# IamArmanNikkhah/viewport-entropy-toolkit

Hardware: NVIDIA B200
Metric: user-frame samples/sec (bin+weighted entropy, 200 tiles) (higher is better)
Workload: dtype f64

## Files before the change

viewport_entropy_toolkit_b200/csrc/vet_whist_i8.cuh:

```cuda
#pragma once
#include <cuda.h>

#include "vet_common.cuh"
#include "vet_stream_tma.cuh"

namespace vet {

constexpr int kI8Slices = 5;
constexpr int kI8FracBits = 39;
constexpr int kI8TilesPerBlock = 48;
constexpr int kI8N = kI8Slices * kI8TilesPerBlock;
constexpr int kI8M = 128;
constexpr int kI8BK = 128;
constexpr int kI8Stages = 3;
constexpr int kI8StagesOne = 4;
constexpr int kI8ABytes = kI8M * kI8BK;
constexpr int kI8BBytes = kI8N * kI8BK;
constexpr int kI8StageBytes = 2 * kI8ABytes + kI8BBytes;
constexpr int kI8Threads = 192;
constexpr int kI8MaxSplit = 8;
constexpr int kI8TmemCols = 512;
constexpr int kI8SmemBytes = kI8Stages * kI8StageBytes + 1024;
static_assert(kI8StageBytes % 1024 == 0 && (kI8ABytes + kI8BBytes) % 1024 == 0, "stages must keep the 1024 B swizzle alignment");
static_assert(kI8StagesOne * (kI8ABytes + kI8BBytes) <= kI8Stages * kI8StageBytes, "both layouts share one ring");

__device__ __forceinline__ void tma_load_2d(uint32_t dst, const void* tmap, uint32_t bar, int c0, int c1) {
  asm volatile(
      "cp.async.bulk.tensor.2d.shared::cluster.global.mbarrier::complete_tx::bytes [%0], [%1, {%3, %4}], [%2];" ::"r"(dst),
      "l"(tmap), "r"(bar), "r"(c0), "r"(c1)
      : "memory");
}
__device__ __forceinline__ void tc_fence_before() { asm volatile("tcgen05.fence::before_thread_sync;" ::: "memory"); }
__device__ __forceinline__ void tc_fence_after() { asm volatile("tcgen05.fence::after_thread_sync;" ::: "memory"); }
__device__ __forceinline__ void tc_alloc(uint32_t smem_dst, uint32_t cols) {
  asm volatile("tcgen05.alloc.cta_group::1.sync.aligned.shared::cta.b32 [%0], %1;" ::"r"(smem_dst), "r"(cols) : "memory");
  asm volatile("tcgen05.relinquish_alloc_permit.cta_group::1.sync.aligned;" ::: "memory");
}
__device__ __forceinline__ void tc_dealloc(uint32_t taddr, uint32_t cols) {
  asm volatile("tcgen05.dealloc.cta_group::1.sync.aligned.b32 %0, %1;" ::"r"(taddr), "r"(cols) : "memory");
}
__device__ __forceinline__ void tc_commit(uint32_t bar) {
  asm volatile("tcgen05.commit.cta_group::1.mbarrier::arrive::one.shared::cluster.b64 [%0];" ::"r"(bar) : "memory");
}
__device__ __forceinline__ void tc_mma_i8(uint32_t d, uint64_t adesc, uint64_t bdesc, uint32_t idesc, uint32_t accumulate) {
  asm volatile(
      "{\n"
      ".reg .pred p;\n"
      "setp.ne.b32 p, %4, 0;\n"
      "tcgen05.mma.cta_group::1.kind::i8 [%0], %1, %2, %3, p;\n"
      "}\n" ::"r"(d),
      "l"(adesc), "l"(bdesc), "r"(idesc), "r"(accumulate)
      : "memory");
}
__device__ __forceinline__ void tc_ld16(uint32_t taddr, uint32_t (&r)[16]) {
  asm volatile(
      "tcgen05.ld.sync.aligned.32x32b.x16.b32 {%0, %1, %2, %3, %4, %5, %6, %7, %8, %9, %10, %11, %12, %13, %14, %15}, [%16];"
      : "=r"(r[0]), "=r"(r[1]), "=r"(r[2]), "=r"(r[3]), "=r"(r[4]), "=r"(r[5]), "=r"(r[6]), "=r"(r[7]), "=r"(r[8]), "=r"(r[9]),
        "=r"(r[10]), "=r"(r[11]), "=r"(r[12]), "=r"(r[13]), "=r"(r[14]), "=r"(r[15])
      : "r"(taddr)
      : "memory");
}
__device__ __forceinline__ void tc_wait_ld() { asm volatile("tcgen05.wait::ld.sync.aligned;" ::: "memory"); }

__device__ __forceinline__ uint64_t i8_smem_desc(uint32_t saddr) {
  return (uint64_t)((saddr & 0x3FFFFu) >> 4) | (1ull << 16) | ((uint64_t)(1024 >> 4) << 32) | (1ull << 46) | (2ull << 61);
}
constexpr uint32_t kI8InstrDesc = (2u << 4) | ((uint32_t)(kI8N >> 3) << 17) | ((uint32_t)(kI8M >> 4) << 24);

struct WhistI8Args {
  int64_t F;
  int T;
  int n_blocks;
  int row_a;
  int row_b;
  const uint32_t* flag_b;
  const uint32_t* run_if;
  int shift;
  int accumulate;
  const int2* kb_range;
  double* hist;
  int ksplit;
  int* part;
};

__global__ void __launch_bounds__(kI8Threads, 1)
k_whist_i8(const __grid_constant__ CUtensorMap tm_cnt, const __grid_constant__ CUtensorMap tm_w, WhistI8Args a) {
  const int tile_id = blockIdx.x / a.ksplit;
  const int sp = blockIdx.x % a.ksplit;
  const int nb = tile_id % a.n_blocks;
  const int mb = tile_id / a.n_blocks;
  if (a.run_if && a.run_if[mb] == 0u) return;
  extern __shared__ unsigned char smem_dyn[];
  __shared__ __align__(8) unsigned long long s_full[kI8StagesOne], s_empty[kI8StagesOne], s_accum;
  __shared__ uint32_t s_tmem;
  const int warp = threadIdx.x >> 5, lane = threadIdx.x & 31;
  const uint32_t ring = (smem_u32(smem_dyn) + 1023u) & ~1023u;
  int2 kr = a.kb_range[nb];
  if (a.ksplit > 1) {
    const int per = (kr.y - kr.x + a.ksplit - 1) / a.ksplit;
    kr.x = min(kr.y, kr.x + sp * per);
    kr.y = min(kr.y, kr.x + per);
  }
  const bool two = a.flag_b && a.flag_b[mb] != 0u;

  const uint32_t nstages = two ? kI8Stages : kI8StagesOne;
  const uint32_t stage_bytes = two ? (uint32_t)kI8StageBytes : (uint32_t)(kI8ABytes + kI8BBytes);
  const uint32_t w_off = two ? 2u * kI8ABytes : (uint32_t)kI8ABytes;
  if (threadIdx.x == 0) {
    for (int i = 0; i < kI8StagesOne; ++i) {
      mbar_init(smem_u32(&s_full[i]), 1);
      mbar_init(smem_u32(&s_empty[i]), 1);
    }
    mbar_init(smem_u32(&s_accum), 1);
    asm volatile("fence.mbarrier_init.release.cluster;" ::: "memory");
  }
  if (warp == 1) tc_alloc(smem_u32(&s_tmem), kI8TmemCols);
  tc_fence_before();
  __syncthreads();
  tc_fence_after();
  const uint32_t tmem = s_tmem;

  if (warp == 0) {
    if (lane == 0) {
      uint32_t stage = 0, phase = 0;
      for (int kb = kr.x; kb < kr.y; ++kb) {
        mbar_wait(smem_u32(&s_empty[stage]), phase ^ 1u);
        const uint32_t bar = smem_u32(&s_full[stage]);
        const uint32_t base = ring + stage * stage_bytes;
        mbar_expect_tx(bar, stage_bytes);
        tma_load_2d(base, &tm_cnt, bar, kb * kI8BK, a.row_a + mb * kI8M);
        if (two) tma_load_2d(base + kI8ABytes, &tm_cnt, bar, kb * kI8BK, a.row_b + mb * kI8M);
        tma_load_2d(base + w_off, &tm_w, bar, kb * kI8BK, nb * kI8N);
        if (++stage == nstages) {
          stage = 0;
          phase ^= 1u;
        }
      }
    }
  } else if (warp == 1) {
    if (lane == 0) {
      uint32_t stage = 0, phase = 0;
      for (int kb = kr.x; kb < kr.y; ++kb) {
        mbar_wait(smem_u32(&s_full[stage]), phase);
        tc_fence_after();
        const uint32_t base = ring + stage * stage_bytes;
#pragma unroll
        for (int k = 0; k < kI8BK / 32; ++k) {
          const uint32_t acc = (kb > kr.x || k > 0) ? 1u : 0u;
          const uint64_t bdesc = i8_smem_desc(base + w_off + k * 32);
          tc_mma_i8(tmem, i8_smem_desc(base + k * 32), bdesc, kI8InstrDesc, acc);
          if (two) tc_mma_i8(tmem + 256, i8_smem_desc(base + kI8ABytes + k * 32), bdesc, kI8InstrDesc, acc);
        }
        tc_commit(smem_u32(&s_empty[stage]));
        if (++stage == nstages) {
          stage = 0;
          phase ^= 1u;
        }
      }
      tc_commit(smem_u32(&s_accum));
    }
    __syncwarp();
  } else {
    const int q = warp & 3;
    const int64_t f = (int64_t)mb * kI8M + q * 32 + lane;
    const uint32_t lane_base = tmem + ((uint32_t)(q * 32) << 16);
    if (a.ksplit > 1) {
      int* __restrict__ part = a.part + ((int64_t)tile_id * a.ksplit + sp) * (2 * kI8N * kI8M) + q * 32 + lane;
      const bool have = kr.y > kr.x;
      if (have) {
        mbar_wait(smem_u32(&s_accum), 0u);
        tc_fence_after();
      }
#pragma unroll 1
      for (int c0 = 0; c0 < kI8N; c0 += 16) {
        uint32_t r0[16], r1[16];
#pragma unroll
        for (int j = 0; j < 16; ++j) r0[j] = r1[j] = 0u;
        if (have) {
          tc_ld16(lane_base + c0, r0);
          if (two) tc_ld16(lane_base + 256 + c0, r1);
          tc_wait_ld();
        }
#pragma unroll
        for (int j = 0; j < 16; ++j) {
          __stcg(part + (c0 + j) * kI8M, (int)r0[j]);
          if (two) __stcg(part + (kI8N + c0 + j) * kI8M, (int)r1[j]);
        }
      }
    } else {
      mbar_wait(smem_u32(&s_accum), 0u);
      tc_fence_after();
#pragma unroll 1
      for (int j0 = 0; j0 < kI8TilesPerBlock; j0 += 16) {
        double v[16];
#pragma unroll
        for (int j = 0; j < 16; ++j) v[j] = 0.0;
#pragma unroll
        for (int s = kI8Slices - 1; s >= 0; --s) {
          uint32_t r0[16], r1[16];
          tc_ld16(lane_base + s * kI8TilesPerBlock + j0, r0);
          if (two) tc_ld16(lane_base + 256 + s * kI8TilesPerBlock + j0, r1);
          tc_wait_ld();
          const double scale = __longlong_as_double((long long)(1023 + 8 * s - kI8FracBits + a.shift) << 52);
#pragma unroll
          for (int j = 0; j < 16; ++j) {
            long long x = (long long)(int)r0[j];
            if (two) x += (long long)(int)r1[j] << 8;
            v[j] = fma((double)x, scale, v[j]);
          }
        }
        if (f < a.F) {
          double* __restrict__ row = a.hist + f * (int64_t)a.T;
#pragma unroll
          for (int j = 0; j < 16; ++j) {
            const int tile = nb * kI8TilesPerBlock + j0 + j;
            if (tile < a.T) row[tile] = a.accumulate ? row[tile] + v[j] : v[j];
          }
        }
      }
    }
  }
  tc_fence_before();
  __syncthreads();
  if (warp == 1) tc_dealloc(tmem, kI8TmemCols);
}

__global__ void __launch_bounds__(kI8M) k_whist_i8_finish(WhistI8Args a) {
  const int tile_id = blockIdx.y;
  const int nb = tile_id % a.n_blocks;
  const int mb = tile_id / a.n_blocks;
  if (a.run_if && a.run_if[mb] == 0u) return;
  const int j = blockIdx.x;
  const int tile = nb * kI8TilesPerBlock + j;
  const int64_t f = (int64_t)mb * kI8M + threadIdx.x;
  if (tile >= a.T || f >= a.F) return;
  const bool two = a.flag_b && a.flag_b[mb] != 0u;
  const int* __restrict__ part = a.part + (int64_t)tile_id * a.ksplit * (2 * kI8N * kI8M) + threadIdx.x;
  int x0[kI8Slices], x1[kI8Slices];
#pragma unroll
  for (int s = 0; s < kI8Slices; ++s) x0[s] = x1[s] = 0;
#pragma unroll
  for (int sp = 0; sp < kI8MaxSplit; ++sp) {
    if (sp < a.ksplit) {
#pragma unroll
      for (int s = 0; s < kI8Slices; ++s) {
        const int* p = part + (int64_t)sp * (2 * kI8N * kI8M) + (s * kI8TilesPerBlock + j) * kI8M;
        x0[s] += __ldcg(p);
        if (two) x1[s] += __ldcg(p + kI8N * kI8M);
      }
    }
  }
  double v = 0.0;
#pragma unroll
  for (int s = kI8Slices - 1; s >= 0; --s) {
    long long x = (long long)x0[s];
    if (two) x += (long long)x1[s] << 8;
    const double scale = __longlong_as_double((long long)(1023 + 8 * s - kI8FracBits + a.shift) << 52);
    v = fma((double)x, scale, v);
  }
  double* __restrict__ row = a.hist + f * (int64_t)a.T;
  row[tile] = a.accumulate ? row[tile] + v : v;
}

struct CntPlanesArgs {
  const uint32_t* cnt;
  int64_t F;
  int cpad;
  int kp;
  int64_t plane_stride;
  uint8_t* planes;
  uint8_t* dirty;
  uint32_t* hi1;
  uint32_t* hi2;
};

__global__ void __launch_bounds__(256) k_cnt_planes(CntPlanesArgs a) {
  const int lane = threadIdx.x & 31;
  const int64_t warp = (blockIdx.x * (int64_t)blockDim.x + threadIdx.x) >> 5;
  const int64_t nwarps = ((int64_t)gridDim.x * blockDim.x) >> 5;
  const int upr = a.kp >> 7;
  const int64_t units = a.F * upr;
  uint32_t* __restrict__ p0 = reinterpret_cast<uint32_t*>(a.planes);
  uint32_t* __restrict__ p1 = reinterpret_cast<uint32_t*>(a.planes + a.plane_stride);
  uint32_t* __restrict__ p2 = reinterpret_cast<uint32_t*>(a.planes + 2 * a.plane_stride);
  constexpr int kUnroll = 4;
  for (int64_t u0 = warp * kUnroll; u0 < units; u0 += nwarps * kUnroll) {
    uint4 v[kUnroll];
#pragma unroll
    for (int i = 0; i < kUnroll; ++i) {
      const int64_t u = u0 + i;
      v[i] = make_uint4(0u, 0u, 0u, 0u);
      if (u < units) {
        const int64_t f = u / upr;
        const int c = (int)(u % upr) * 128 + lane * 4;
        if (c < a.cpad) v[i] = __ldg(reinterpret_cast<const uint4*>(a.cnt + f * (int64_t)a.cpad + c));
      }
    }
#pragma unroll
    for (int i = 0; i < kUnroll; ++i) {
      const int64_t u = u0 + i;
      if (u < units) {
        const int64_t f = u / upr;
        const int64_t o = (f * (int64_t)a.kp + (u % upr) * 128) / 4 + lane;
        const uint32_t w1 = pack_bytes(v[i], 8), w2 = pack_bytes(v[i], 16);
        p0[o] = pack_bytes(v[i], 0);
        p1[o] = w1;
        p2[o] = w2;
        if (w1 && *reinterpret_cast<volatile uint32_t*>(&a.hi1[f >> 7]) == 0u) atomicOr(&a.hi1[f >> 7], 1u);
        if (w2 && *reinterpret_cast<volatile uint32_t*>(&a.hi2[f >> 7]) == 0u) atomicOr(&a.hi2[f >> 7], 1u);
        if (u % upr == 0 && lane == 0) a.dirty[f] = 3;
      }
    }
  }
}

}
```

Measured before the change: 418.8 billion.

## Use variable-width tile blocks with sparse k-lists and fused high-plane pass

Replaces fixed 48-tile blocks with per-block descriptors of variable width (up to 51 tiles, N up to 256), choosing a matching weight tensor map per width. K-blocks now come from a sparse kb_list so empty k-chunks are skipped. The high-byte plane is handled as a second pass inside the same kernel, with a TMEM-free barrier, instead of a separate launch with run_if/accumulate. It also adds an optional globaltimer instrumentation path. The cost is per-element tcgen05 loads for unaligned columns and more complex synchronisation.

```diff
diff --git a/viewport_entropy_toolkit_b200/csrc/vet_whist_i8.cuh b/viewport_entropy_toolkit_b200/csrc/vet_whist_i8.cuh
--- a/viewport_entropy_toolkit_b200/csrc/vet_whist_i8.cuh
+++ b/viewport_entropy_toolkit_b200/csrc/vet_whist_i8.cuh
@@ -9,20 +9,33 @@
 constexpr int kI8Slices = 5;
 constexpr int kI8FracBits = 39;
 constexpr int kI8TilesPerBlock = 48;
-constexpr int kI8N = kI8Slices * kI8TilesPerBlock;
+constexpr int kI8MaxTiles = 51;
+constexpr int kI8MaxN = 256;
 constexpr int kI8M = 128;
 constexpr int kI8BK = 128;
 constexpr int kI8Stages = 3;
 constexpr int kI8StagesOne = 4;
 constexpr int kI8ABytes = kI8M * kI8BK;
-constexpr int kI8BBytes = kI8N * kI8BK;
+constexpr int kI8BBytes = kI8MaxN * kI8BK;
 constexpr int kI8StageBytes = 2 * kI8ABytes + kI8BBytes;
 constexpr int kI8Threads = 192;
 constexpr int kI8MaxSplit = 8;
 constexpr int kI8TmemCols = 512;
+constexpr int kI8PartPlane = kI8MaxN * kI8M;
 constexpr int kI8SmemBytes = kI8Stages * kI8StageBytes + 1024;
 static_assert(kI8StageBytes % 1024 == 0 && (kI8ABytes + kI8BBytes) % 1024 == 0, "stages must keep the 1024 B swizzle alignment");
 static_assert(kI8StagesOne * (kI8ABytes + kI8BBytes) <= kI8Stages * kI8StageBytes, "both layouts share one ring");
+static_assert(((kI8Slices * kI8MaxTiles + 15) & ~15) == kI8MaxN, "the widest block fills N = 256");
+
+#ifdef VET_WHIST_I8_CLOCK
+constexpr int kI8ClockSlots = 4096;
+__device__ unsigned long long g_whist_i8_clock[kI8ClockSlots][3];
+__device__ __forceinline__ unsigned long long globaltimer() {
+  unsigned long long t;
+  asm volatile("mov.u64 %0, %globaltimer;" : "=l"(t));
+  return t;
+}
+#endif
 
 __device__ __forceinline__ void tma_load_2d(uint32_t dst, const void* tmap, uint32_t bar, int c0, int c1) {
   asm volatile(
@@ -61,47 +74,73 @@
       : "memory");
 }
 __device__ __forceinline__ void tc_wait_ld() { asm volatile("tcgen05.wait::ld.sync.aligned;" ::: "memory"); }
+__device__ __forceinline__ void tc_ld16_any(uint32_t taddr, uint32_t (&r)[16]) {
+  if ((taddr & 15u) == 0u) {
+    tc_ld16(taddr, r);
+  } else {
+#pragma unroll
+    for (int j = 0; j < 16; ++j)
+      asm volatile("tcgen05.ld.sync.aligned.32x32b.x1.b32 {%0}, [%1];" : "=r"(r[j]) : "r"(taddr + j) : "memory");
+  }
+}
 
 __device__ __forceinline__ uint64_t i8_smem_desc(uint32_t saddr) {
   return (uint64_t)((saddr & 0x3FFFFu) >> 4) | (1ull << 16) | ((uint64_t)(1024 >> 4) << 32) | (1ull << 46) | (2ull << 61);
 }
-constexpr uint32_t kI8InstrDesc = (2u << 4) | ((uint32_t)(kI8N >> 3) << 17) | ((uint32_t)(kI8M >> 4) << 24);
+__device__ __forceinline__ uint32_t i8_instr_desc(int n) {
+  return (2u << 4) | ((uint32_t)(n >> 3) << 17) | ((uint32_t)(kI8M >> 4) << 24);
+}
+
+struct I8WeightMaps {
+  CUtensorMap m[kI8MaxN / 16];
+};
+
+struct I8Block {
+  int first, nt, w_row, kb;
+};
 
 struct WhistI8Args {
   int64_t F;
   int T;
   int n_blocks;
-  int row_a;
-  int row_b;
-  const uint32_t* flag_b;
-  const uint32_t* run_if;
-  int shift;
-  int accumulate;
-  const int2* kb_range;
+  int plane_rows;
+  const uint32_t* hi1;
+  const uint32_t* hi2;
+  const I8Block* blocks;
+  const int* kb_list;
   double* hist;
   int ksplit;
   int* part;
 };
 
+__device__ __forceinline__ double i8_scale(int s, int shift) {
+  return __longlong_as_double((long long)(1023 + 8 * s - kI8FracBits + shift) << 52);
+}
+
 __global__ void __launch_bounds__(kI8Threads, 1)
-k_whist_i8(const __grid_constant__ CUtensorMap tm_cnt, const __grid_constant__ CUtensorMap tm_w, WhistI8Args a) {
+k_whist_i8(const __grid_constant__ CUtensorMap tm_cnt, const __grid_constant__ I8WeightMaps tm_w, WhistI8Args a) {
+#ifdef VET_WHIST_I8_CLOCK
+  if (threadIdx.x == 0 && blockIdx.x < kI8ClockSlots) g_whist_i8_clock[blockIdx.x][0] = globaltimer();
+#endif
   const int tile_id = blockIdx.x / a.ksplit;
   const int sp = blockIdx.x % a.ksplit;
   const int nb = tile_id % a.n_blocks;
   const int mb = tile_id / a.n_blocks;
-  if (a.run_if && a.run_if[mb] == 0u) return;
   extern __shared__ unsigned char smem_dyn[];
-  __shared__ __align__(8) unsigned long long s_full[kI8StagesOne], s_empty[kI8StagesOne], s_accum;
+  __shared__ __align__(8) unsigned long long s_full[kI8StagesOne], s_empty[kI8StagesOne], s_accum, s_tfree;
   __shared__ uint32_t s_tmem;
   const int warp = threadIdx.x >> 5, lane = threadIdx.x & 31;
   const uint32_t ring = (smem_u32(smem_dyn) + 1023u) & ~1023u;
-  int2 kr = a.kb_range[nb];
+  const I8Block blk = a.blocks[nb];
+  const int n = (kI8Slices * blk.nt + 15) & ~15;
+  int k0 = blk.kb, k1 = a.blocks[nb + 1].kb;
   if (a.ksplit > 1) {
-    const int per = (kr.y - kr.x + a.ksplit - 1) / a.ksplit;
-    kr.x = min(kr.y, kr.x + sp * per);
-    kr.y = min(kr.y, kr.x + per);
-  }
-  const bool two = a.flag_b && a.flag_b[mb] != 0u;
+    const int per = (k1 - k0 + a.ksplit - 1) / a.ksplit;
+    k0 = min(k1, k0 + sp * per);
+    k1 = min(k1, k0 + per);
+  }
+  const bool two = a.hi1[mb] != 0u;
+  const int passes = a.hi2[mb] != 0u ? 2 : 1;
 
   const uint32_t nstages = two ? kI8Stages : kI8StagesOne;
   const uint32_t stage_bytes = two ? (uint32_t)kI8StageBytes : (uint32_t)(kI8ABytes + kI8BBytes);
@@ -112,6 +151,7 @@
       mbar_init(smem_u32(&s_empty[i]), 1);
     }
     mbar_init(smem_u32(&s_accum), 1);
+    mbar_init(smem_u32(&s_tfree), 4);
     asm volatile("fence.mbarrier_init.release.cluster;" ::: "memory");
   }
   if (warp == 1) tc_alloc(smem_u32(&s_tmem), kI8TmemCols);
@@ -122,131 +162,162 @@
 
   if (warp == 0) {
     if (lane == 0) {
+      const CUtensorMap* tmw = &tm_w.m[n / 16 - 1];
       uint32_t stage = 0, phase = 0;
-      for (int kb = kr.x; kb < kr.y; ++kb) {
-        mbar_wait(smem_u32(&s_empty[stage]), phase ^ 1u);
-        const uint32_t bar = smem_u32(&s_full[stage]);
-        const uint32_t base = ring + stage * stage_bytes;
-        mbar_expect_tx(bar, stage_bytes);
-        tma_load_2d(base, &tm_cnt, bar, kb * kI8BK, a.row_a + mb * kI8M);
-        if (two) tma_load_2d(base + kI8ABytes, &tm_cnt, bar, kb * kI8BK, a.row_b + mb * kI8M);
-        tma_load_2d(base + w_off, &tm_w, bar, kb * kI8BK, nb * kI8N);
-        if (++stage == nstages) {
-          stage = 0;
-          phase ^= 1u;
+      for (int pass = 0; pass < passes; ++pass) {
+        const bool b = pass == 0 && two;
+        const uint32_t bytes = (b ? 2u * kI8ABytes : (uint32_t)kI8ABytes) + (uint32_t)n * kI8BK;
+        const int row_a = (pass == 0 ? 0 : 2 * a.plane_rows) + mb * kI8M;
+        for (int i = k0; i < k1; ++i) {
+          const int kc = a.kb_list[i] * kI8BK;
+          mbar_wait(smem_u32(&s_empty[stage]), phase ^ 1u);
+          const uint32_t bar = smem_u32(&s_full[stage]);
+          const uint32_t base = ring + stage * stage_bytes;
+          mbar_expect_tx(bar, bytes);
+          tma_load_2d(base, &tm_cnt, bar, kc, row_a);
+          if (b) tma_load_2d(base + kI8ABytes, &tm_cnt, bar, kc, a.plane_rows + mb * kI8M);
+          tma_load_2d(base + w_off, tmw, bar, kc, blk.w_row);
+          if (++stage == nstages) {
+            stage = 0;
+            phase ^= 1u;
+          }
         }
       }
     }
   } else if (warp == 1) {
     if (lane == 0) {
+      const uint32_t idesc = i8_instr_desc(n);
       uint32_t stage = 0, phase = 0;
-      for (int kb = kr.x; kb < kr.y; ++kb) {
-        mbar_wait(smem_u32(&s_full[stage]), phase);
-        tc_fence_after();
-        const uint32_t base = ring + stage * stage_bytes;
-#pragma unroll
-        for (int k = 0; k < kI8BK / 32; ++k) {
-          const uint32_t acc = (kb > kr.x || k > 0) ? 1u : 0u;
-          const uint64_t bdesc = i8_smem_desc(base + w_off + k * 32);
-          tc_mma_i8(tmem, i8_smem_desc(base + k * 32), bdesc, kI8InstrDesc, acc);
-          if (two) tc_mma_i8(tmem + 256, i8_smem_desc(base + kI8ABytes + k * 32), bdesc, kI8InstrDesc, acc);
-        }
-        tc_commit(smem_u32(&s_empty[stage]));
-        if (++stage == nstages) {
-          stage = 0;
-          phase ^= 1u;
-        }
-      }
-      tc_commit(smem_u32(&s_accum));
+      for (int pass = 0; pass < passes; ++pass) {
+        const bool b = pass == 0 && two;
+        if (pass == 1) {
+          mbar_wait(smem_u32(&s_tfree), 0u);
+          tc_fence_after();
+        }
+        for (int i = k0; i < k1; ++i) {
+          mbar_wait(smem_u32(&s_full[stage]), phase);
+          tc_fence_after();
+          const uint32_t base = ring + stage * stage_bytes;
+#pragma unroll
+          for (int k = 0; k < kI8BK / 32; ++k) {
+            const uint32_t acc = (i > k0 || k > 0) ? 1u : 0u;
+            const uint64_t bdesc = i8_smem_desc(base + w_off + k * 32);
+            tc_mma_i8(tmem, i8_smem_desc(base + k * 32), bdesc, idesc, acc);
+            if (b) tc_mma_i8(tmem + 256, i8_smem_desc(base + kI8ABytes + k * 32), bdesc, idesc, acc);
+          }
+          tc_commit(smem_u32(&s_empty[stage]));
+          if (++stage == nstages) {
+            stage = 0;
+            phase ^= 1u;
+          }
+        }
+        tc_commit(smem_u32(&s_accum));
+      }
     }
     __syncwarp();
   } else {
     const int q = warp & 3;
     const int64_t f = (int64_t)mb * kI8M + q * 32 + lane;
     const uint32_t lane_base = tmem + ((uint32_t)(q * 32) << 16);
-    if (a.ksplit > 1) {
-      int* __restrict__ part = a.part + ((int64_t)tile_id * a.ksplit + sp) * (2 * kI8N * kI8M) + q * 32 + lane;
-      const bool have = kr.y > kr.x;
+    const bool have = k1 > k0;
+#pragma unroll 1
+    for (int pass = 0; pass < passes; ++pass) {
+      const bool b = pass == 0 && two;
       if (have) {
-        mbar_wait(smem_u32(&s_accum), 0u);
+        mbar_wait(smem_u32(&s_accum), (uint32_t)pass);
         tc_fence_after();
       }
+      if (a.ksplit > 1) {
+        int* __restrict__ part =
+            a.part + ((int64_t)tile_id * a.ksplit + sp) * (3 * kI8PartPlane) + pass * 2 * kI8PartPlane + q * 32 + lane;
 #pragma unroll 1
-      for (int c0 = 0; c0 < kI8N; c0 += 16) {
-        uint32_t r0[16], r1[16];
-#pragma unroll
-        for (int j = 0; j < 16; ++j) r0[j] = r1[j] = 0u;
-        if (have) {
-          tc_ld16(lane_base + c0, r0);
-          if (two) tc_ld16(lane_base + 256 + c0, r1);
-          tc_wait_ld();
-        }
-#pragma unroll
-        for (int j = 0; j < 16; ++j) {
-          __stcg(part + (c0 + j) * kI8M, (int)r0[j]);
-          if (two) __stcg(part + (kI8N + c0 + j) * kI8M, (int)r1[j]);
-        }
-      }
-    } else {
-      mbar_wait(smem_u32(&s_accum), 0u);
-      tc_fence_after();
+        for (int c0 = 0; c0 < n; c0 += 16) {
+          uint32_t r0[16], r1[16];
+#pragma unroll
+          for (int j = 0; j < 16; ++j) r0[j] = r1[j] = 0u;
+          if (have) {
+            tc_ld16(lane_base + c0, r0);
+            if (b) tc_ld16(lane_base + 256 + c0, r1);
+            tc_wait_ld();
+          }
+#pragma unroll
+          for (int j = 0; j < 16; ++j) {
+            __stcg(part + (c0 + j) * kI8M, (int)r0[j]);
+            if (b) __stcg(part + (kI8PartPlane + (c0 + j) * kI8M), (int)r1[j]);
+          }
+        }
+      } else {
 #pragma unroll 1
-      for (int j0 = 0; j0 < kI8TilesPerBlock; j0 += 16) {
-        double v[16];
-#pragma unroll
-        for (int j = 0; j < 16; ++j) v[j] = 0.0;
-#pragma unroll
-        for (int s = kI8Slices - 1; s >= 0; --s) {
-          uint32_t r0[16], r1[16];
-          tc_ld16(lane_base + s * kI8TilesPerBlock + j0, r0);
-          if (two) tc_ld16(lane_base + 256 + s * kI8TilesPerBlock + j0, r1);
-          tc_wait_ld();
-          const double scale = __longlong_as_double((long long)(1023 + 8 * s - kI8FracBits + a.shift) << 52);
-#pragma unroll
-          for (int j = 0; j < 16; ++j) {
-            long long x = (long long)(int)r0[j];
-            if (two) x += (long long)(int)r1[j] << 8;
-            v[j] = fma((double)x, scale, v[j]);
-          }
-        }
-        if (f < a.F) {
-          double* __restrict__ row = a.hist + f * (int64_t)a.T;
-#pragma unroll
-          for (int j = 0; j < 16; ++j) {
-            const int tile = nb * kI8TilesPerBlock + j0 + j;
-            if (tile < a.T) row[tile] = a.accumulate ? row[tile] + v[j] : v[j];
-          }
-        }
+        for (int j0 = 0; j0 < blk.nt; j0 += 16) {
+          const int c = max(0, min(j0, blk.nt - 16));
+          double v[16];
+#pragma unroll
+          for (int j = 0; j < 16; ++j) v[j] = 0.0;
+#pragma unroll
+          for (int s = kI8Slices - 1; s >= 0; --s) {
+            uint32_t r0[16], r1[16];
+            tc_ld16_any(lane_base + s * blk.nt + c, r0);
+            if (b) tc_ld16_any(lane_base + 256 + s * blk.nt + c, r1);
+            tc_wait_ld();
+            const double scale = i8_scale(s, 16 * pass);
+#pragma unroll
+            for (int j = 0; j < 16; ++j) {
+              long long x = (long long)(int)r0[j];
+              if (b) x += (long long)(int)r1[j] << 8;
+              v[j] = fma((double)x, scale, v[j]);
+            }
+          }
+          if (f < a.F) {
+            double* __restrict__ row = a.hist + f * (int64_t)a.T + blk.first;
+#pragma unroll
+            for (int j = 0; j < 16; ++j) {
+              const int t = c + j;
+              if (t >= j0 && t < blk.nt) row[t] = pass ? row[t] + v[j] : v[j];
+            }
+          }
+        }
+      }
+      if (pass + 1 < passes) {
+        tc_fence_before();
+        __syncwarp();
+        if (lane == 0) mbar_arrive(smem_u32(&s_tfree));
       }
     }
   }
   tc_fence_before();
   __syncthreads();
   if (warp == 1) tc_dealloc(tmem, kI8TmemCols);
+#ifdef VET_WHIST_I8_CLOCK
+  if (threadIdx.x == 0 && blockIdx.x < kI8ClockSlots) {
+    g_whist_i8_clock[blockIdx.x][1] = globaltimer();
+    g_whist_i8_clock[blockIdx.x][2] = (unsigned long long)((k1 - k0) | n << 16 | (int)two << 28 | (passes - 1) << 29);
+  }
+#endif
 }
 
 __global__ void __launch_bounds__(kI8M) k_whist_i8_finish(WhistI8Args a) {
   const int tile_id = blockIdx.y;
   const int nb = tile_id % a.n_blocks;
   const int mb = tile_id / a.n_blocks;
-  if (a.run_if && a.run_if[mb] == 0u) return;
+  const I8Block blk = a.blocks[nb];
   const int j = blockIdx.x;
-  const int tile = nb * kI8TilesPerBlock + j;
   const int64_t f = (int64_t)mb * kI8M + threadIdx.x;
-  if (tile >= a.T || f >= a.F) return;
-  const bool two = a.flag_b && a.flag_b[mb] != 0u;
-  const int* __restrict__ part = a.part + (int64_t)tile_id * a.ksplit * (2 * kI8N * kI8M) + threadIdx.x;
-  int x0[kI8Slices], x1[kI8Slices];
-#pragma unroll
-  for (int s = 0; s < kI8Slices; ++s) x0[s] = x1[s] = 0;
+  if (j >= blk.nt || f >= a.F) return;
+  const bool two = a.hi1[mb] != 0u;
+  const bool hi = a.hi2[mb] != 0u;
+  const int* __restrict__ part = a.part + (int64_t)tile_id * a.ksplit * (3 * kI8PartPlane) + threadIdx.x;
+  int x0[kI8Slices], x1[kI8Slices], x2[kI8Slices];
+#pragma unroll
+  for (int s = 0; s < kI8Slices; ++s) x0[s] = x1[s] = x2[s] = 0;
 #pragma unroll
   for (int sp = 0; sp < kI8MaxSplit; ++sp) {
     if (sp < a.ksplit) {
 #pragma unroll
       for (int s = 0; s < kI8Slices; ++s) {
-        const int* p = part + (int64_t)sp * (2 * kI8N * kI8M) + (s * kI8TilesPerBlock + j) * kI8M;
+        const int* p = part + (int64_t)sp * (3 * kI8PartPlane) + (s * blk.nt + j) * kI8M;
         x0[s] += __ldcg(p);
-        if (two) x1[s] += __ldcg(p + kI8N * kI8M);
+        if (two) x1[s] += __ldcg(p + kI8PartPlane);
+        if (hi) x2[s] += __ldcg(p + 2 * kI8PartPlane);
       }
     }
   }
@@ -255,11 +326,15 @@
   for (int s = kI8Slices - 1; s >= 0; --s) {
     long long x = (long long)x0[s];
     if (two) x += (long long)x1[s] << 8;
-    const double scale = __longlong_as_double((long long)(1023 + 8 * s - kI8FracBits + a.shift) << 52);
-    v = fma((double)x, scale, v);
-  }
-  double* __restrict__ row = a.hist + f * (int64_t)a.T;
-  row[tile] = a.accumulate ? row[tile] + v : v;
+    v = fma((double)x, i8_scale(s, 0), v);
+  }
+  if (hi) {
+    double v2 = 0.0;
+#pragma unroll
+    for (int s = kI8Slices - 1; s >= 0; --s) v2 = fma((double)x2[s], i8_scale(s, 16), v2);
+    v = v + v2;
+  }
+  a.hist[f * (int64_t)a.T + blk.first + j] = v;
 }
 
 struct CntPlanesArgs {
```

New measurement: 428.5 billion, median of 6. +2.3%, better.
